# taki0112/vit-tensorflow

Hardware: AMD Instinct MI355X
Metric: images/sec (fwd+bwd) ViT-B/16 224px bf16 (higher is better)
Workload: dtype bf16; 1 GPU; vit_b16_224 fwd+bwd, batch 256/GPU, N(0,1) NHWC images resident in HBM, random-init weights, softmax-CE cotangent, dropout 0; global_batch=256, parallelism=dp1, compute=bf16

## Files before the change

### vit-tensorflow_amd/csrc/gemm_bf16.hip

```cpp
#include <array>
#include <map>
#include <mutex>

#include "gemm_bf16_common.h"

static int g_allow_320 = 1;
static int g_shared_gpu = 0;
int gemm_bf16_pick(int M, int N);

namespace {

template <int BM, int BN, int WM, int WN, int MODE, bool LDS_EPI, int SCHED>
__global__ __launch_bounds__(WM * WN * 64) void gemm_bf16_nt_kernel(Bf16GemmArgs g, EpiParams ep, int tiles_m, int tiles_n,
                                                                    int kt_per_split) {
  constexpr int NW = WM * WN;
  constexpr int WTM = BM / WM, WTN = BN / WN;
  constexpr int MT = WTM / 32, NT = WTN / 32;
  constexpr int A_BYTES = BM * BK * 2, B_BYTES = BN * BK * 2, STAGE = A_BYTES + B_BYTES;
  constexpr int A_INSTR = BM / 8 / NW, B_INSTR = BN / 8 / NW;
  static_assert(BM % (8 * NW) == 0 && BN % (8 * NW) == 0, "tile rows must split evenly over the waves");
  extern __shared__ __attribute__((aligned(16))) char smem[];

  const int nwg = gridDim.x, bid = blockIdx.x;
  const int xcd = bid & 7, q8 = nwg >> 3, r8 = nwg & 7;
// ... 8 lines not shown
  const int wave = __builtin_amdgcn_readfirstlane(tid >> 6);
  const int wm = wave / WN, wn = wave - wm * WN;

  if (g.stagger > 0 && bid < 256 && blockIdx.y == 0) {
    const int ph = (bid >> 3) & 3;
    for (int i = 0; i < ph * g.stagger; ++i) __builtin_amdgcn_s_sleep(32);
  }

  int offA[A_INSTR], offB[B_INSTR];
#pragma unroll
  for (int i = 0; i < A_INSTR; ++i) {
    const int row = (i * NW + wave) * 8 + (lane >> 3);
    const int c = (lane & 7) ^ ((row >> 1) & 7);
    offA[i] = row * (int)g.lda + c * 8;
  }
#pragma unroll
  for (int i = 0; i < B_INSTR; ++i) {
    const int row = (i * NW + wave) * 8 + (lane >> 3);
    const int c = (lane & 7) ^ ((row >> 1) & 7);
    offB[i] = row * (int)g.ldb + c * 8;
  }
  auto stage_ptr = [&](int buf, const bf16_t* Ap, const bf16_t* Bp, int kt) {
    char* base = smem + buf * STAGE;
#pragma unroll
    for (int i = 0; i < A_INSTR; ++i)
      __builtin_amdgcn_global_load_lds((gbl_void_t*)(Ap + (offA[i] + kt * BK)),
                                       (lds_void_t*)(base + (i * NW + wave) * 1024), 16, 0, 0);
#pragma unroll
    for (int i = 0; i < B_INSTR; ++i)
      __builtin_amdgcn_global_load_lds((gbl_void_t*)(Bp + (offB[i] + kt * BK)),
                                       (lds_void_t*)(base + A_BYTES + (i * NW + wave) * 1024), 16, 0, 0);
  };

  const int sw = ((lane & 31) >> 1) & 7;
  const int a_row_byte = (wm * WTM + (lane & 31)) * 128;
  const int b_row_byte = A_BYTES + (wn * WTN + (lane & 31)) * 128;
  const int khalf = lane >> 5;
  const bool has_bias = ep.bias != nullptr, has_scale = ep.scale != nullptr;
  const int64_t out_off = (int64_t)z * ep.partial_stride;

  int it = 0;
  int logical = logical0;
  if (logical >= total_tiles) return;
  const int gm = (tiles_n >= 8 ? 4 : 1) * (g.reverse_m ? -1 : 1);
  int tile_m, tile_n;
  decode_tile(logical, tiles_m, tiles_n, gm, tile_m, tile_n);
  const bf16_t* Ag = g.A + (int64_t)tile_m * BM * g.lda + (int64_t)kt0 * BK;
  const bf16_t* Bg = g.B + (int64_t)tile_n * BN * g.ldb + (int64_t)kt0 * BK;
  if (SCHED == 2 && nk > 0) stage_ptr(0, Ag, Bg, 0);

  for (;;) {
    auto stage = [&](int buf, int kt) { stage_ptr(buf, Ag, Bg, kt); };
    const int next_logical = logical + nwg;
    const bool has_next = SCHED == 2 && next_logical < total_tiles;
    int ntm = 0, ntn = 0;
    if (has_next) decode_tile(next_logical, tiles_m, tiles_n, gm, ntm, ntn);
    const bf16_t* Agn = g.A + (int64_t)ntm * BM * g.lda + (int64_t)kt0 * BK;
    const bf16_t* Bgn = g.B + (int64_t)ntn * BN * g.ldb + (int64_t)kt0 * BK;

    f32x16 acc[MT][NT];
#pragma unroll
    for (int i = 0; i < MT; ++i)
#pragma unroll
      for (int j = 0; j < NT; ++j)
#pragma unroll
        for (int r = 0; r < 16; ++r) acc[i][j][r] = 0.f;

    {
      if (SCHED != 2 && nk > 0) stage(0, 0);
      for (int kt = 0; kt < nk; ++kt) {
        asm volatile("s_waitcnt vmcnt(0)" ::: "memory");
        __syncthreads();
        if (kt + 1 < nk) stage((it + 1) & 1, kt + 1);
        else if (has_next) stage_ptr((it + 1) & 1, Agn, Bgn, 0);
        const char* base = smem + (it & 1) * STAGE;
#pragma unroll
        for (int ks = 0; ks < BK / 16; ++ks) {
          const int cb = ((ks * 2 + khalf) ^ sw) << 4;
          bf16x8 af[MT], bfr[NT];
#pragma unroll
          for (int i = 0; i < MT; ++i) af[i] = *(const bf16x8*)(base + a_row_byte + i * 32 * 128 + cb);
#pragma unroll
          for (int j = 0; j < NT; ++j) bfr[j] = *(const bf16x8*)(base + b_row_byte + j * 32 * 128 + cb);
#pragma unroll
          for (int i = 0; i < MT; ++i)
#pragma unroll
            for (int j = 0; j < NT; ++j)
              acc[i][j] = __builtin_amdgcn_mfma_f32_32x32x16_bf16(bfr[j], af[i], acc[i][j], 0, 0, 0);
        }
        ++it;
      }
    }

    const bool interior = epilogue_fast_ok(ep, MODE) && (tile_m + 1) * BM <= ep.M && (tile_n + 1) * BN <= ep.N;
    constexpr int RR = ((SCHED == 2 && 64 * (BN + 4) * 4 > STAGE) || (MT % 2 != 0)) ? 32 : 64;
    if constexpr (LDS_EPI) {
      constexpr int SROW = BN + 4;
      constexpr int LPRW = BN / 4, RPIW = 64 / LPRW;
      constexpr int RPW = RR / (NW * RPIW);
      static_assert(RPW >= 1 && RR * SROW * 4 <= (SCHED == 2 ? 1 : 2) * STAGE, "staging round must fit the free pipeline buffer(s)");
      float* st = (float*)(smem + (SCHED == 2 ? ((it + 1) & 1) * STAGE : 0));
      const int col_l = (lane % LPRW) * 4;
      const int gcol = tile_n * BN + col_l;
      float4 b4 = make_float4(0.f, 0.f, 0.f, 0.f), s4 = make_float4(1.f, 1.f, 1.f, 1.f);
      if (interior && has_bias) b4 = *(const float4*)(ep.bias + gcol);
      if (interior && has_scale) s4 = *(const float4*)(ep.scale + gcol);
      float4 cs = make_float4(0.f, 0.f, 0.f, 0.f);
      auto cs_add = [&](float4 r) { if (MODE == EPI_GELU_BWD) { cs.x += r.x; cs.y += r.y; cs.z += r.z; cs.w += r.w; } };
#pragma clang loop unroll(full)
      for (int R = 0; R < BM / RR; ++R) {
        const int wm_r = (R * RR) / WTM, i0 = ((R * RR) % WTM) / 32;
        __syncthreads();
        if (wm == wm_r) {
#pragma unroll
          for (int ii = 0; ii < RR / 32; ++ii)
#pragma unroll
            for (int j = 0; j < NT; ++j)
#pragma unroll
              for (int q = 0; q < 4; ++q)
                *(float4*)(st + (ii * 32 + (lane & 31)) * SROW + wn * WTN + j * 32 + 8 * q + 4 * khalf) =
                    make_float4(acc[i0 + ii][j][4 * q], acc[i0 + ii][j][4 * q + 1], acc[i0 + ii][j][4 * q + 2], acc[i0 + ii][j][4 * q + 3]);
        }
        __syncthreads();
        float4 v[RPW];
#pragma unroll
        for (int k = 0; k < RPW; ++k) v[k] = *(const float4*)(st + ((k * NW + wave) * RPIW + lane / LPRW) * SROW + col_l);
        const int grow0 = tile_m * BM + R * RR + lane / LPRW;
        if (interior) {
          float4 x[RPW];
#pragma unroll
          for (int k = 0; k < RPW; ++k) x[k] = epilogue_fast_load<MODE, bf16_t>(ep, grow0 + (k * NW + wave) * RPIW, gcol);
          if (MODE == EPI_BIAS_RESID && has_scale) {
#pragma unroll
            for (int k = 0; k < RPW; ++k) {
              if (has_bias) epilogue_fast4<MODE, bf16_t, true, true>(ep, grow0 + (k * NW + wave) * RPIW, gcol, v[k], b4, s4, x[k], out_off);
              else epilogue_fast4<MODE, bf16_t, false, true>(ep, grow0 + (k * NW + wave) * RPIW, gcol, v[k], b4, s4, x[k], out_off);
            }
          } else if (has_bias) {
#pragma unroll
            for (int k = 0; k < RPW; ++k) cs_add(epilogue_fast4<MODE, bf16_t, true, false>(ep, grow0 + (k * NW + wave) * RPIW, gcol, v[k], b4, s4, x[k], out_off));
          } else {
#pragma unroll
            for (int k = 0; k < RPW; ++k) cs_add(epilogue_fast4<MODE, bf16_t, false, false>(ep, grow0 + (k * NW + wave) * RPIW, gcol, v[k], b4, s4, x[k], out_off));
          }
        } else {
#pragma unroll
          for (int k = 0; k < RPW; ++k) cs_add(epilogue_apply4<MODE, bf16_t>(ep, grow0 + (k * NW + wave) * RPIW, gcol, v[k], out_off));
        }
      }
      if (MODE == EPI_GELU_BWD && ep.colsum != nullptr) {
        __syncthreads();
        *(float4*)(st + (wave * RPIW + lane / LPRW) * BN + col_l) = cs;
        __syncthreads();
        if (tid < BN) {
          float a = 0.f;
#pragma unroll
          for (int w = 0; w < NW * RPIW; ++w) a += st[w * BN + tid];
          const int c = tile_n * BN + tid;
          if (c < ep.N) ep.colsum[(int64_t)tile_m * ep.ldcs + c] = a;
        }
      }
      if (SCHED == 2) __syncthreads();
    } else {
      const int row0 = tile_m * BM + wm * WTM + (lane & 31);
      const int col00 = tile_n * BN + wn * WTN + 4 * khalf;
      if (interior) {
        auto run = [&](auto hb, auto hs) {
          constexpr bool HB = decltype(hb)::value, HS = decltype(hs)::value;
#pragma unroll
          for (int j = 0; j < NT; ++j)
#pragma unroll
            for (int qp = 0; qp < 2; ++qp) {
              float4 b4[2], s4[2], x[2][MT];
#pragma unroll
              for (int qq = 0; qq < 2; ++qq) {
                const int col = col00 + j * 32 + 8 * (2 * qp + qq);
                b4[qq] = HB ? *(const float4*)(ep.bias + col) : make_float4(0.f, 0.f, 0.f, 0.f);
                s4[qq] = HS ? *(const float4*)(ep.scale + col) : make_float4(1.f, 1.f, 1.f, 1.f);
#pragma unroll
                for (int i = 0; i < MT; ++i) x[qq][i] = epilogue_fast_load<MODE, bf16_t>(ep, row0 + i * 32, col);
              }
#pragma unroll
              for (int qq = 0; qq < 2; ++qq) {
                const int q = 2 * qp + qq;
                const int col = col00 + j * 32 + 8 * q;
#pragma unroll
                for (int i = 0; i < MT; ++i)
                  epilogue_fast4<MODE, bf16_t, HB, HS>(ep, row0 + i * 32, col,
                                                       make_float4(acc[i][j][4 * q], acc[i][j][4 * q + 1], acc[i][j][4 * q + 2], acc[i][j][4 * q + 3]),
                                                       b4[qq], s4[qq], x[qq][i], out_off);
              }
            }
        };
        if (has_bias && has_scale) run(std::true_type{}, std::true_type{});
        else if (has_bias) run(std::true_type{}, std::false_type{});
        else run(std::false_type{}, std::false_type{});
      } else {
#pragma unroll
        for (int i = 0; i < MT; ++i) {
#pragma unroll
          for (int j = 0; j < NT; ++j) {
#pragma unroll
            for (int q = 0; q < 4; ++q)
              epilogue_apply4<MODE, bf16_t>(ep, row0 + i * 32, col00 + j * 32 + 8 * q,
                                            make_float4(acc[i][j][4 * q], acc[i][j][4 * q + 1], acc[i][j][4 * q + 2], acc[i][j][4 * q + 3]),
                                            out_off);
          }
        }
      }
    }

    if (!has_next) break;
    logical = next_logical;
    tile_m = ntm; tile_n = ntn;
    Ag = Agn; Bg = Bgn;
  }
}

template <int BM, int BN, int WM, int WN, int MODE, bool LDS_EPI, int SCHED = 0>
void launch_variant(const Bf16GemmArgs& g, const EpiParams& ep, hipStream_t s) {
  constexpr int SMEM = 2 * (BM + BN) * BK * 2;
  static_assert(64 * (BN + 4) * 4 <= SMEM, "epilogue staging must fit in the pipeline buffers");
  auto kern = gemm_bf16_nt_kernel<BM, BN, WM, WN, MODE, LDS_EPI, SCHED>;
  vitx_set_max_smem((const void*)kern, SMEM);
  const int tiles_m = (int)ceil_div(g.M, BM), tiles_n = (int)ceil_div(g.N, BN);
  const int nk = g.K / BK;
  const int split = g.split_k > 1 ? g.split_k : 1;
  const int per = (int)ceil_div(nk, split);
  const int zs = (int)ceil_div(nk, per);
  const unsigned gx = (SCHED == 2 && zs == 1) ? (unsigned)std::min(tiles_m * tiles_n, 256) : (unsigned)(tiles_m * tiles_n);
  dim3 grid(gx, (unsigned)zs), block(WM * WN * 64);
  hipLaunchKernelGGL(kern, grid, block, SMEM, s, g, ep, tiles_m, tiles_n, per);
}

template <int MODE>
void launch_mode(const Bf16GemmArgs& g, const EpiParams& ep, hipStream_t s) {
  int k = g.kernel & 15;
  if (k == 0) k = gemm_bf16_pick(g.M, g.N);
  const bool bf16_out = (MODE == EPI_STORE || MODE == EPI_BIAS_GELU || MODE == EPI_GELU_BWD);
// ... 188 lines not shown
```

### vit-tensorflow_amd/csrc/gemm_bf16_common.h

```cpp
#pragma once
#include <algorithm>
#include <cstdio>
#include <cstdlib>
#include <type_traits>
#include <utility>

#include "kernels.h"

namespace {

typedef __attribute__((address_space(3))) void lds_void_t;
typedef const __attribute__((address_space(1))) void gbl_void_t;

constexpr int BK = 64;

template <typename F, int... I>
__device__ __forceinline__ void static_for_impl(F&& f, std::integer_sequence<int, I...>) { (f(std::integral_constant<int, I>{}), ...); }
template <int N, typename F>
__device__ __forceinline__ void static_for(F&& f) { static_for_impl(f, std::make_integer_sequence<int, N>{}); }
template <int V> using ic = std::integral_constant<int, V>;

__device__ __forceinline__ void decode_tile_fwd(int L, int tiles_m, int tiles_n, int gm, int& tm, int& tn);
__device__ __forceinline__ void decode_tile(int L, int tiles_m, int tiles_n, int gm, int& tm, int& tn) {
  if (gm < 0) { decode_tile_fwd(L, tiles_m, tiles_n, -gm, tm, tn); tm = tiles_m - 1 - tm; return; }
  decode_tile_fwd(L, tiles_m, tiles_n, gm, tm, tn);
}
__device__ __forceinline__ void decode_tile_fwd(int L, int tiles_m, int tiles_n, int gm, int& tm, int& tn) {
  if (gm == 1) { tm = L / tiles_n; tn = L - tm * tiles_n; return; }
  const int group = gm * tiles_n;
  const int gid = L / group, first = gid * gm;
  const int gsz = min(tiles_m - first, gm);
  const int w = L - gid * group;
  tn = w / gsz;
  tm = first + (w - tn * gsz);
}

}

void launch_gemm_bf16_pipe(int variant, int mode, const Bf16GemmArgs& g, const EpiParams& ep, hipStream_t s);
int gemm_bf16_shared_gpu();
void launch_gemm_bf16_persistent_lockstep(int bm, int mode, const Bf16GemmArgs& g, const EpiParams& ep, hipStream_t s);
```

### vit-tensorflow_amd/csrc/gemm_bf16_pipe.hip

```cpp
#include "gemm_bf16_common.h"

#include <cmath>
#include <cstring>
#include <map>
#include <mutex>
#include <vector>

namespace {

__device__ __forceinline__ int wp_lane() {
  int l;
  asm volatile("v_mbcnt_lo_u32_b32 %0, -1, 0\n\tv_mbcnt_hi_u32_b32 %0, -1, %0" : "=v"(l));
  return l;
}

template <int POL>
__device__ __forceinline__ void wp_store16(bf16_t* base, uint32_t elem_off, bf16x8 v) {
  if constexpr (POL == 1) __builtin_nontemporal_store(v, (bf16x8*)(base + elem_off));
  else *(bf16x8*)(base + elem_off) = v;
}

constexpr int GT_LO = (127 - 12) << 7, GT_NE = ((127 + 3) << 7) - GT_LO, GT_BYTES = 2 * GT_NE * 4;
const uint32_t* gelu_table_dev() {
  static std::mutex mu;
  static std::map<int, const uint32_t*> per_dev;
  int dev = 0;
  (void)hipGetDevice(&dev);
  std::lock_guard<std::mutex> lk(mu);
  auto it = per_dev.find(dev);
  if (it != per_dev.end()) return it->second;
  std::vector<uint32_t> h((size_t)2 * GT_NE);
  auto f32_to_bf16 = [](float f) { uint32_t u; memcpy(&u, &f, 4); u += 0x7fffu + ((u >> 16) & 1u); return (uint16_t)(u >> 16); };
  auto f32_to_f16 = [](float f) { _Float16 hh = (_Float16)f; uint16_t u; memcpy(&u, &hh, 2); return u; };
  for (int sgn = 0; sgn < 2; ++sgn)
    for (int t = 0; t < GT_NE; ++t) {
      const uint32_t bits = ((uint32_t)sgn << 31) | ((uint32_t)(t + GT_LO) << 16);
      float xf; memcpy(&xf, &bits, 4);
      const double x = xf, phi = 0.5 * (1.0 + erf(x * 0.70710678118654752440)), gd = phi + x * 0.39894228040143267794 * exp(-0.5 * x * x);
      h[(size_t)sgn * GT_NE + t] = ((uint32_t)f32_to_f16((float)phi) << 16) | f32_to_bf16((float)gd);
    }
  uint32_t* d = nullptr;
  if (hipMalloc((void**)&d, GT_BYTES) != hipSuccess || hipMemcpy(d, h.data(), GT_BYTES, hipMemcpyHostToDevice) != hipSuccess) d = nullptr;
  per_dev[dev] = d;
  return d;
}

// ... 46 lines not shown
  for (int i = 0; i < B_INSTR; ++i) {
    const int row = (wave * B_INSTR + i) * 8 + (lane >> 3);
    offB[i] = (uint32_t)(row * (int)g.ldb + (((lane & 7) ^ ((row >> 1) & 7)) << 3)) * 2u - (uint32_t)((i & 3) * 1024);
  }

  const int gm = ((tiles_n >= 8 && g.stagger != 8) ? 4 : 1) * (g.reverse_m ? -1 : 1);
  auto tile_of = [&](int idx, int& tm, int& tn) {
    if (xw) {
      decode_tile_fwd(idx, w_nr, tiles_n, 8, tm, tn);
      tm += w_r0;
      if (g.reverse_m) tm = tiles_m - 1 - tm;
    } else {
      decode_tile(idx, tiles_m, tiles_n, gm, tm, tn);
    }
  };
  int i_logical = w_first, i_k = 0, issued = 0;
  bool i_more = nk > 0;
  const i32x4 rsA = vitx_make_rsrc(g.A), rsB = vitx_make_rsrc(g.B);
  const uint32_t lds_wa = vitx_lds_addr(smem) + (uint32_t)wave * (A_INSTR * 1024u);
  const uint32_t lds_wb = vitx_lds_addr(smem) + A_BYTES + (uint32_t)wave * (B_INSTR * 1024u);
  uint32_t a_soff = 0, b_soff = 0;
  auto i_set_tile = [&]() {
    int tm, tn;
    tile_of(i_logical, tm, tn);
    a_soff = (uint32_t)(((int64_t)tm * BM * g.lda + (int64_t)kt0 * BK) * 2);
    b_soff = (uint32_t)(((int64_t)tn * BN * g.ldb + (int64_t)kt0 * BK) * 2);
    {
      a_soff = (uint32_t)__builtin_amdgcn_readfirstlane((int)a_soff);
      b_soff = (uint32_t)__builtin_amdgcn_readfirstlane((int)b_soff);
    }
  };
  i_set_tile();
  constexpr int P = A_INSTR + B_INSTR;
  constexpr int N3 = (P + 2) / 3;
  constexpr int N0 = (P + 1) / 3;
  constexpr int N1 = P - N3 - N0;
  bool pending = false;
  const int xp = g.stagger;
  auto issue_piece = [&](uint32_t base, auto p_c) {
    constexpr int p = decltype(p_c)::value;
    const uint32_t sa = a_soff + i_k * (BK * 2), sb = b_soff + i_k * (BK * 2), lb = base;
    if constexpr (p < A_INSTR) {
      if constexpr ((p & 3) == 0) vitx_dma16(rsA, lds_wa + lb + p * 1024, offA[p], sa);
      else vitx_dma16_cont<(p & 3) * 1024>(rsA, offA[p], sa);
    } else {
      constexpr int q = p - A_INSTR;
      if constexpr ((q & 3) == 0) vitx_dma16(rsB, lds_wb + lb + q * 1024, offB[q], sb);
      else vitx_dma16_cont<(q & 3) * 1024>(rsB, offB[q], sb);
    }
  };
  auto i_advance = [&]() {
    ++issued;
    if (++i_k == nk) {
      i_k = 0;
      i_logical += w_stride;
      i_more = persistent && i_logical < w_limit;
      if (i_more) i_set_tile();
    }
  };
  auto issue = [&]() {
    if (!i_more) return;
    const uint32_t base = (issued & 1) * STAGE;
    static_for<P>([&](auto p_c) { issue_piece(base, p_c); });
    i_advance();
  };

  const int sw = ((lane & 31) >> 1) & 7;
  const int a_row_byte = (wm * WTM + (lane & 31)) * 128;
  const int b_row_byte = A_BYTES + (wn * WTN + (lane & 31)) * 128;
  const int khalf = lane >> 5;
  bf16x8 fa[2][MT], fb[2][NT];
  auto load_frags = [&](bf16x8(&af)[MT], bf16x8(&bfr)[NT], const char* base, int ks) {
    const int cb = ((ks * 2 + khalf) ^ sw) << 4;
#pragma unroll
    for (int i = 0; i < MT; ++i) af[i] = *(const bf16x8*)(base + a_row_byte + i * 32 * 128 + cb);
#pragma unroll
    for (int j = 0; j < NT; ++j) bfr[j] = *(const bf16x8*)(base + b_row_byte + j * 32 * 128 + cb);
  };
  constexpr int Q = MT * NT;
  f32x16 acc[MT][NT];
  auto mfma_range = [&](auto cur_c, auto first_c, auto last_c) {
    constexpr int CUR = decltype(cur_c)::value, FIRST = decltype(first_c)::value, LAST = decltype(last_c)::value;
    static_for<(LAST > FIRST ? LAST - FIRST : 0)>([&](auto d) {
      constexpr int idx = FIRST + decltype(d)::value, i = idx / NT, j = idx % NT;
      acc[i][j] = __builtin_amdgcn_mfma_f32_32x32x16_bf16(fb[CUR][j], fa[CUR][i], acc[i][j], 0, 0, 0);
    });
  };
  auto handover = [&]() {
    if (xp & 1) __builtin_amdgcn_s_waitcnt(0xC07F);
    else __builtin_amdgcn_s_waitcnt(0x0070);
    __builtin_amdgcn_s_barrier();
    asm volatile("" ::: "memory");
  };
  const bool has_bias = ep.bias != nullptr, has_scale = ep.scale != nullptr;
  const int64_t out_off = (int64_t)z * ep.partial_stride;

  issue();
  issue();
  constexpr bool GTAB = MODE == EPI_BIAS_GELU && BM == 256;
  if constexpr (GTAB) {
    if (gelu_tab != nullptr) {
      uint32_t* t = (uint32_t*)(smem + 2 * STAGE);
      for (int i = tid; i < 2 * GT_NE; i += NW * 64) t[i] = gelu_tab[i];
    }
  }
  handover();
  load_frags(fa[0], fb[0], smem, 0);
  int it = 0;
  int tile_idx = 0;
#ifndef VITX_GEMM_STAMPS_BUILD
#define VITX_GEMM_STAMPS_BUILD 0
#endif
  constexpr bool kStamps = VITX_GEMM_STAMPS_BUILD != 0;
  auto stamp = [&](int k) {
    if constexpr (kStamps)
      if (g.stamps && tid == 0 && bid < 512 && tile_idx < 15) {
        g.stamps[((int64_t)bid * 16 + tile_idx) * 4 + k] = __builtin_readcyclecounter();
        if (tile_idx == 0 && k == 0)
          g.stamps[((int64_t)bid * 16 + 15) * 4] = ((unsigned long long)__builtin_amdgcn_s_getreg((31 << 11) | 20) << 32) | (unsigned)__builtin_amdgcn_s_getreg((31 << 11) | 4);
      }
  };
  for (int logical = w_first;; logical += w_stride, ++tile_idx) {
    int tile_m, tile_n;
    tile_of(logical, tile_m, tile_n);
    const bool has_next = persistent && logical + w_stride < w_limit;
    stamp(0);
#pragma unroll
    for (int i = 0; i < MT; ++i)
#pragma unroll
      for (int j = 0; j < NT; ++j)
#pragma unroll
        for (int r = 0; r < 16; ++r) acc[i][j][r] = 0.f;

    for (int kt = 0; kt < nk; ++kt) {
      const char* base = smem + (it & 1) * STAGE;
      static_for<BK / 16>([&](auto ks_c) {
        constexpr int ks = decltype(ks_c)::value, CUR = ks & 1;
        constexpr int NP = ks == 3 ? N3 : (ks == 0 ? N0 : (ks == 1 ? N1 : 0));
        constexpr int FP = ks == 3 ? 0 : (ks == 0 ? N3 : N3 + N0);
        if constexpr (ks + 1 < BK / 16) {
          mfma_range(ic<CUR>{}, ic<0>{}, ic<2>{});
          __builtin_amdgcn_sched_barrier(0);
          if (!(xp & 4)) load_frags(fa[CUR ^ 1], fb[CUR ^ 1], base, ks + 1);
        } else {
          handover();
          mfma_range(ic<CUR>{}, ic<0>{}, ic<2>{});
          __builtin_amdgcn_sched_barrier(0);
          if (kt + 1 < nk && !(xp & 4)) load_frags(fa[0], fb[0], smem + ((it + 1) & 1) * STAGE, 0);
          pending = i_more && kt + 1 < nk && !(xp & 2);
        }
        __builtin_amdgcn_sched_barrier(0);
        if constexpr (NP > 0) {
          const uint32_t ibase = (issued & 1) * STAGE;
          static_for<NP>([&](auto d_c) {
            constexpr int d = decltype(d_c)::value;
            mfma_range(ic<CUR>{}, ic<(2 + d < Q ? 2 + d : Q)>{}, ic<(3 + d < Q ? 3 + d : Q)>{});
            if (pending) issue_piece(ibase, ic<FP + d>{});
            __builtin_amdgcn_sched_barrier(0);
          });
          mfma_range(ic<CUR>{}, ic<(2 + NP < Q ? 2 + NP : Q)>{}, ic<Q>{});
          if constexpr (FP + NP == P) {
            if (pending) i_advance();
            pending = false;
          }
        } else {
          mfma_range(ic<CUR>{}, ic<2>{}, ic<Q>{});
        }
        __builtin_amdgcn_sched_barrier(0);
      });
      ++it;
    }

    stamp(1);
    bool wp_done = false;
    {
      const bool interior = epilogue_fast_ok(ep, MODE) && (tile_m + 1) * BM <= ep.M && (tile_n + 1) * BN <= ep.N;
      static_assert((BM == 256 || BM == 320 || BM == 192) && A_INSTR >= 4 && B_INSTR == 4 && WTN == 64 && MT * 32 == WTM && NT == 2, "wave-private epilogue: 256 / 320 x 256 tiles, 2 x 4 waves");
      if constexpr (MODE == EPI_STORE || MODE == EPI_BIAS_GELU || MODE == EPI_BIAS_RESID || MODE == EPI_GELU_BWD) {
        const bool wp_ok = interior && (MODE == EPI_BIAS_RESID || ep.wide_ok) && !(MODE == EPI_STORE && has_bias);
        if (wp_ok) {
          wp_done = true;
          char* const sa = smem + ((it + 1) & 1) * STAGE + wave * (A_INSTR * 1024);
          char* const sb = smem + ((it + 1) & 1) * STAGE + A_BYTES + wave * (B_INSTR * 1024);
          const int le = wp_lane();
          const int m = le & 31, swm = (m >> 1) & 7, kh = le >> 5;
          const int row_w = tile_m * BM + wm * WTM, col_w = tile_n * BN + wn * WTN;
          auto to_bf16x4 = [](float a, float b, float c, float d) { bf16x4 o; o[0] = (bf16_t)a; o[1] = (bf16_t)b; o[2] = (bf16_t)c; o[3] = (bf16_t)d; return o; };
          auto stage_f32 = [&](auto i_c) {
            constexpr int i0 = decltype(i_c)::value;
#pragma unroll
            for (int q = 0; q < 4; ++q) {
              const int ch = 2 * q + kh;
              *(float4*)(sa + m * 128 + ((ch ^ swm) << 4)) = make_float4(acc[i0][0][4 * q], acc[i0][0][4 * q + 1], acc[i0][0][4 * q + 2], acc[i0][0][4 * q + 3]);
              *(float4*)(sb + (m ^ 1) * 128 + ((ch ^ swm ^ 1) << 4)) = make_float4(acc[i0][1][4 * q], acc[i0][1][4 * q + 1], acc[i0][1][4 * q + 2], acc[i0][1][4 * q + 3]);
            }
          };
          if constexpr (MODE == EPI_STORE) {
            bf16_t* const outp = (bf16_t*)ep.out + out_off + (int64_t)row_w * ep.ldo + col_w;
            const uint32_t ldo = (uint32_t)ep.ldo, ooff = (uint32_t)(le >> 3) * ldo + (uint32_t)(le & 7) * 8u;
            auto run = [&](auto nt_c) {
              constexpr int POL = decltype(nt_c)::value;
              static_for<MT>([&](auto i_c) {
                constexpr int i0 = decltype(i_c)::value;
                char* const ar = (i0 & 1) ? sb : sa;
#pragma unroll
                for (int j = 0; j < NT; ++j)
#pragma unroll
                  for (int q = 0; q < 4; ++q)
                    *(bf16x4*)(ar + m * 128 + (((j * 4 + q) ^ swm) << 4) + kh * 8) =
                        to_bf16x4(acc[i0][j][4 * q], acc[i0][j][4 * q + 1], acc[i0][j][4 * q + 2], acc[i0][j][4 * q + 3]);
                bf16x8 v[4];
#pragma unroll
                for (int k = 0; k < 4; ++k) {
                  const int r = k * 8 + (le >> 3);
                  v[k] = *(const bf16x8*)(ar + r * 128 + (((le & 7) ^ ((r >> 1) & 7)) << 4));
                }
#pragma unroll
                for (int k = 0; k < 4; ++k) wp_store16<POL>(outp, ooff + (uint32_t)(i0 * 32 + k * 8) * ldo, v[k]);
              });
            };
            if (ep.nt_out) run(ic<1>{});
            else run(ic<0>{});
          } else if constexpr (MODE == EPI_BIAS_GELU) {
            const float* const bias_w = has_bias ? ep.bias + col_w + 4 * kh : nullptr;
            bf16_t* const o1 = (bf16_t*)ep.out + (int64_t)row_w * ep.ldo + col_w;
            bf16_t* const o2 = (bf16_t*)ep.out2 + (int64_t)row_w * ep.ldo2 + col_w;
            const uint32_t ldo = (uint32_t)ep.ldo, ldo2 = (uint32_t)ep.ldo2;
            const uint32_t o1off = (uint32_t)(le >> 3) * ldo + (uint32_t)(le & 7) * 8u, o2off = (uint32_t)(le >> 3) * ldo2 + (uint32_t)(le & 7) * 8u;
            const bool use_tab = GTAB && gelu_tab != nullptr;
            const char* const gt = smem + 2 * STAGE;
            auto run = [&](auto nt_c, auto tab_c) {
              constexpr int POL = decltype(nt_c)::value;
              constexpr bool TAB = decltype(tab_c)::value;
              static_for<MT>([&](auto i_c) {
                constexpr int i0 = decltype(i_c)::value;
#pragma unroll
                for (int j = 0; j < NT; ++j) {
                  float4 bzj[4];
#pragma unroll
                  for (int q = 0; q < 4; ++q) bzj[q] = bias_w ? *(const float4*)(bias_w + j * 32 + 8 * q) : make_float4(0.f, 0.f, 0.f, 0.f);
#pragma unroll
                  for (int q = 0; q < 4; ++q) {
                    const bf16x4 h = to_bf16x4(acc[i0][j][4 * q] + bzj[q].x, acc[i0][j][4 * q + 1] + bzj[q].y, acc[i0][j][4 * q + 2] + bzj[q].z,
                                               acc[i0][j][4 * q + 3] + bzj[q].w);
                    const int off = m * 128 + (((j * 4 + q) ^ swm) << 4) + kh * 8;
                    if constexpr (TAB) {
                      const uint32_t p0 = __builtin_bit_cast(uint2, h).x, p1 = __builtin_bit_cast(uint2, h).y;
                      auto look = [&](uint32_t bits15, uint32_t sign) {
                        const int t = min(max((int)bits15 - GT_LO, 0), GT_NE - 1);
                        return *(const uint32_t*)(gt + ((uint32_t)t + sign * GT_NE) * 4u);
                      };
                      const uint32_t e0 = look(p0 & 0x7fffu, (p0 >> 15) & 1u), e1 = look((p0 >> 16) & 0x7fffu, p0 >> 31);
                      const uint32_t e2 = look(p1 & 0x7fffu, (p1 >> 15) & 1u), e3 = look((p1 >> 16) & 0x7fffu, p1 >> 31);
                      auto phi = [](uint32_t e) { return (float)__builtin_bit_cast(_Float16, (uint16_t)(e >> 16)); };
                      const float x0 = __builtin_bit_cast(float, p0 << 16), x1 = __builtin_bit_cast(float, p0 & 0xffff0000u);
                      const float x2 = __builtin_bit_cast(float, p1 << 16), x3 = __builtin_bit_cast(float, p1 & 0xffff0000u);
                      uint2 gdw;
                      gdw.x = __builtin_amdgcn_perm(e1, e0, 0x05040100u);
                      gdw.y = __builtin_amdgcn_perm(e3, e2, 0x05040100u);
                      *(uint2*)(sa + off) = gdw;
                      *(bf16x4*)(sb + off) = to_bf16x4(x0 * phi(e0), x1 * phi(e1), x2 * phi(e2), x3 * phi(e3));
                    } else {
                      float4 g, gd;
                      gelu_both4(make_float4((float)h[0], (float)h[1], (float)h[2], (float)h[3]), g, gd);
                      *(bf16x4*)(sa + off) = to_bf16x4(gd.x, gd.y, gd.z, gd.w);
                      *(bf16x4*)(sb + off) = to_bf16x4(g.x, g.y, g.z, g.w);
                    }
                  }
                }
                bf16x8 vd[4], vg[4];
#pragma unroll
                for (int k = 0; k < 4; ++k) {
                  const int r = k * 8 + (le >> 3);
                  const int off = r * 128 + (((le & 7) ^ ((r >> 1) & 7)) << 4);
                  vd[k] = *(const bf16x8*)(sa + off);
                  vg[k] = *(const bf16x8*)(sb + off);
                }
#pragma unroll
                for (int k = 0; k < 4; ++k) {
                  wp_store16<POL>(o1, o1off + (uint32_t)(i0 * 32 + k * 8) * ldo, vd[k]);
                  wp_store16<0>(o2, o2off + (uint32_t)(i0 * 32 + k * 8) * ldo2, vg[k]);
                }
              });
            };
            if constexpr (GTAB) {
              if (use_tab) { if (ep.nt_out) run(ic<1>{}, std::true_type{}); else run(ic<0>{}, std::true_type{}); }
              else if (ep.nt_out) run(ic<1>{}, std::false_type{});
              else run(ic<0>{}, std::false_type{});
            } else {
              if (ep.nt_out) run(ic<1>{}, std::false_type{});
              else run(ic<0>{}, std::false_type{});
            }
          } else if constexpr (MODE == EPI_BIAS_RESID) {
            const int c16 = le & 15, ar1 = c16 >> 3;
            const uint32_t lr = (uint32_t)(le >> 4), lc = (uint32_t)c16 * 4u;
            const float4 bb = has_bias ? *(const float4*)(ep.bias + col_w + lc) : make_float4(0.f, 0.f, 0.f, 0.f);
            const float4 ss = has_scale ? *(const float4*)(ep.scale + col_w + lc) : make_float4(1.f, 1.f, 1.f, 1.f);
            const char* const rb = ar1 ? sb : sa;
            const float* const rp = ep.resid + (int64_t)row_w * ep.ldr + col_w;
// ... 49 lines not shown
                const char* rowp = rb + (r ^ ar1) * 128;
                const int swr = ((r >> 1) & 7) ^ ar1;
                va[k] = *(const float4*)(rowp + ((ch0 ^ swr) << 4));
                vb[k] = *(const float4*)(rowp + (((ch0 + 1) ^ swr) << 4));
              }
#pragma unroll
              for (int k = 0; k < 4; ++k) {
                const float4 a = va[k], b = vb[k];
                const bf16x8 o = pack_bf16x8(make_float4(a.x * (float)x[k][0], a.y * (float)x[k][1], a.z * (float)x[k][2], a.w * (float)x[k][3]),
                                             make_float4(b.x * (float)x[k][4], b.y * (float)x[k][5], b.z * (float)x[k][6], b.w * (float)x[k][7]));
                wp_store16<0>(op, ooff + (uint32_t)(i0 * 32 + k * 8) * ldo, o);
                cs.x += (float)o[0]; cs.y += (float)o[1]; cs.z += (float)o[2]; cs.w += (float)o[3];
                cs2.x += (float)o[4]; cs2.y += (float)o[5]; cs2.z += (float)o[6]; cs2.w += (float)o[7];
              }
            });
            if (ep.colsum != nullptr) {
              auto red = [&](float v) { v += __shfl_xor(v, 8); v += __shfl_xor(v, 16); v += __shfl_xor(v, 32); return v; };
              cs.x = red(cs.x); cs.y = red(cs.y); cs.z = red(cs.z); cs.w = red(cs.w);
              cs2.x = red(cs2.x); cs2.y = red(cs2.y); cs2.z = red(cs2.z); cs2.w = red(cs2.w);
              if (le < 8) {
                float* crow = ep.colsum + (int64_t)(tile_m * 2 + wm) * ep.ldcs + col_w + lc;
                *(float4*)crow = cs;
                *(float4*)(crow + 4) = cs2;
              }
            }
          }
        }
      }
      {
        if (!wp_done) {
          const int le = wp_lane();
          char* const sa = smem + ((it + 1) & 1) * STAGE + wave * (A_INSTR * 1024);
          char* const sb = smem + ((it + 1) & 1) * STAGE + A_BYTES + wave * (B_INSTR * 1024);
          const int m = le & 31, swm = (m >> 1) & 7, kh = le >> 5;
          const int row_w = tile_m * BM + wm * WTM, col_w = tile_n * BN + wn * WTN;
          const int c16 = le & 15, ar1 = c16 >> 3, lr = le >> 4, gcolr = col_w + c16 * 4;
          const char* const rb = ar1 ? sb : sa;
          float4 cs = make_float4(0.f, 0.f, 0.f, 0.f);
          static_for<MT>([&](auto i_c) {
            constexpr int i0 = decltype(i_c)::value;
#pragma unroll
            for (int q = 0; q < 4; ++q) {
              const int ch = 2 * q + kh;
              *(float4*)(sa + m * 128 + ((ch ^ swm) << 4)) = make_float4(acc[i0][0][4 * q], acc[i0][0][4 * q + 1], acc[i0][0][4 * q + 2], acc[i0][0][4 * q + 3]);
              *(float4*)(sb + (m ^ 1) * 128 + ((ch ^ swm ^ 1) << 4)) = make_float4(acc[i0][1][4 * q], acc[i0][1][4 * q + 1], acc[i0][1][4 * q + 2], acc[i0][1][4 * q + 3]);
            }
#pragma unroll 2
            for (int k = 0; k < 8; ++k) {
              const int r = k * 4 + lr;
              const float4 v = *(const float4*)(rb + (r ^ ar1) * 128 + ((((c16 & 7) ^ ((r >> 1) & 7)) ^ ar1) << 4));
              const float4 res = epilogue_apply4<MODE, bf16_t>(ep, row_w + i0 * 32 + r, gcolr, v, out_off);
              if (MODE == EPI_GELU_BWD) { cs.x += res.x; cs.y += res.y; cs.z += res.z; cs.w += res.w; }
            }
          });
          if (MODE == EPI_GELU_BWD && ep.colsum != nullptr) {
            auto red = [&](float v) { v += __shfl_xor(v, 16); v += __shfl_xor(v, 32); return v; };
            cs.x = red(cs.x); cs.y = red(cs.y); cs.z = red(cs.z); cs.w = red(cs.w);
            if (le < 16 && gcolr < ep.N) {
              float* crow = ep.colsum + (int64_t)(tile_m * 2 + wm) * ep.ldcs + gcolr;
              if (gcolr + 3 < ep.N) *(float4*)crow = cs;
              else { crow[0] = cs.x; if (gcolr + 1 < ep.N) crow[1] = cs.y; if (gcolr + 2 < ep.N) crow[2] = cs.z; }
            }
          }
        }
      }

    }
    stamp(2);
    if (!has_next) break;
    __builtin_amdgcn_s_waitcnt(0xC07F);
    asm volatile("" ::: "memory");
    issue();
    load_frags(fa[0], fb[0], smem + (it & 1) * STAGE, 0);
    stamp(3);
  }
}

template <int BM, int BN, int WM, int WN, int MODE>
void launch_pipe(const Bf16GemmArgs& g, const EpiParams& ep, hipStream_t s, bool one_tile_per_wg = false) {
  constexpr int SMEM = 2 * (BM + BN) * BK * 2 + ((MODE == EPI_BIAS_GELU && BM == 256) ? GT_BYTES : 0);
  if (((int64_t)ceil_div(g.M, BM) * BM * g.lda + g.K) * 2 >= (1LL << 31) || ((int64_t)ceil_div(g.N, BN) * BN * g.ldb + g.K) * 2 >= (1LL << 31)) {
    launch_gemm_bf16_persistent_lockstep(BM, MODE, g, ep, s);
    return;
  }
  auto kern = gemm_bf16_nt_pipe_kernel<BM, BN, WM, WN, MODE>;
  vitx_set_max_smem((const void*)kern, SMEM);
  const int tiles_m = (int)ceil_div(g.M, BM), tiles_n = (int)ceil_div(g.N, BN);
  const int nk = g.K / BK;
  const int split = g.split_k > 1 ? g.split_k : 1;
  const int per = (int)ceil_div(nk, split);
  const int zs = (int)ceil_div(nk, per);
  static const int phase_env = [] { const char* v = vitx_env("VITX_GEMM_PHASE"); return v ? atoi(v) : 0; }();
  Bf16GemmArgs gp = g;
  if (gp.phase == 0) gp.phase = phase_env;
  static const int walk_env = [] { const char* v = vitx_env("VITX_GEMM_WALK"); return v ? atoi(v) : -1; }();
  static const int grid_cap = [] { const char* v = vitx_env("VITX_GEMM_GRID"); return v ? atoi(v) : 256 * (WM * WN == 4 ? 2 : 1); }();
  const unsigned gx = (zs == 1 && !gemm_bf16_shared_gpu() && !g.shared_gpu && !one_tile_per_wg) ? (unsigned)std::min(tiles_m * tiles_n, grid_cap) : (unsigned)(tiles_m * tiles_n);
  dim3 grid(gx, (unsigned)zs), block(WM * WN * 64);
  const bool walk2_ok = BM == 256 && zs == 1 && gx == (unsigned)grid_cap && (gx & 7) == 0 && gx < (unsigned)(tiles_m * tiles_n) && tiles_n >= 8 && tiles_m >= 64 && g.stagger != 8;
  gp.walk = (walk2_ok && walk_env != 0) ? 2 : 0;
  const uint32_t* gtab = (MODE == EPI_BIAS_GELU && BM == 256 && gelu_table_on()) ? gelu_table_dev() : nullptr;
  hipLaunchKernelGGL(kern, grid, block, SMEM, s, gp, ep, tiles_m, tiles_n, per, gtab);
}

template <int MODE>
void pipe_mode(int variant, const Bf16GemmArgs& g, const EpiParams& ep, hipStream_t s) {
// ... 25 lines not shown
```

Before: 7620 images/sec.

## Switch bf16 NT GEMM kernels from 32x32x16 to 16x16x32 MFMA

Replaces the 32x32x16 bf16 MFMA instruction with 16x16x32 MFMA in both the basic and pipelined NT GEMM kernels. Each 32x32 accumulator is kept as four 16x16 sub-blocks, and LDS fragment loads are recomputed for 16-row groups with a quarter-K lane split. The pipelined kernel's interleaving of global-to-LDS pieces and fragment reloads is rescheduled around two half passes over the tile. Epilogue and staging offsets now go through an acc_pos abstraction for the new accumulator layout. The aim is higher MFMA throughput or better latency hiding, at the cost of more LDS reads per K step, more issue slots, and schedule complexity.

```diff
diff --git a/vit-tensorflow_amd/csrc/gemm_bf16.hip b/vit-tensorflow_amd/csrc/gemm_bf16.hip
--- a/vit-tensorflow_amd/csrc/gemm_bf16.hip
+++ b/vit-tensorflow_amd/csrc/gemm_bf16.hip
@@ -64,10 +64,10 @@
                                        (lds_void_t*)(base + A_BYTES + (i * NW + wave) * 1024), 16, 0, 0);
   };
 
-  const int sw = ((lane & 31) >> 1) & 7;
-  const int a_row_byte = (wm * WTM + (lane & 31)) * 128;
-  const int b_row_byte = A_BYTES + (wn * WTN + (lane & 31)) * 128;
-  const int khalf = lane >> 5;
+  const int sw = ((lane & 15) >> 1) & 7;
+  const int a_row_byte = (wm * WTM + (lane & 15)) * 128;
+  const int b_row_byte = A_BYTES + (wn * WTN + (lane & 15)) * 128;
+  const int kq = lane >> 4;
   const bool has_bias = ep.bias != nullptr, has_scale = ep.scale != nullptr;
   const int64_t out_off = (int64_t)z * ep.partial_stride;
 
@@ -106,20 +106,19 @@
         if (kt + 1 < nk) stage((it + 1) & 1, kt + 1);
         else if (has_next) stage_ptr((it + 1) & 1, Agn, Bgn, 0);
         const char* base = smem + (it & 1) * STAGE;
-#pragma unroll
-        for (int ks = 0; ks < BK / 16; ++ks) {
-          const int cb = ((ks * 2 + khalf) ^ sw) << 4;
-          bf16x8 af[MT], bfr[NT];
-#pragma unroll
-          for (int i = 0; i < MT; ++i) af[i] = *(const bf16x8*)(base + a_row_byte + i * 32 * 128 + cb);
-#pragma unroll
-          for (int j = 0; j < NT; ++j) bfr[j] = *(const bf16x8*)(base + b_row_byte + j * 32 * 128 + cb);
-#pragma unroll
-          for (int i = 0; i < MT; ++i)
-#pragma unroll
-            for (int j = 0; j < NT; ++j)
-              acc[i][j] = __builtin_amdgcn_mfma_f32_32x32x16_bf16(bfr[j], af[i], acc[i][j], 0, 0, 0);
-        }
+        static_for<BK / 32>([&](auto ks_c) {
+          constexpr int ks = decltype(ks_c)::value;
+          const int cb = ((ks * 4 + kq) ^ sw) << 4;
+          bf16x8 af[2 * MT], bfr[2 * NT];
+#pragma unroll
+          for (int i = 0; i < 2 * MT; ++i) af[i] = *(const bf16x8*)(base + a_row_byte + i * 16 * 128 + cb);
+#pragma unroll
+          for (int j = 0; j < 2 * NT; ++j) bfr[j] = *(const bf16x8*)(base + b_row_byte + j * 16 * 128 + cb);
+          static_for<4 * MT * NT>([&](auto d) {
+            constexpr int b16 = decltype(d)::value / (2 * NT), j16 = decltype(d)::value % (2 * NT);
+            mfma_item<(b16 & 1) * 2 + (j16 & 1)>(acc[b16 >> 1][j16 >> 1], bfr[j16], af[b16]);
+          });
+        });
         ++it;
       }
     }
@@ -149,9 +148,10 @@
 #pragma unroll
             for (int j = 0; j < NT; ++j)
 #pragma unroll
-              for (int q = 0; q < 4; ++q)
-                *(float4*)(st + (ii * 32 + (lane & 31)) * SROW + wn * WTN + j * 32 + 8 * q + 4 * khalf) =
-                    make_float4(acc[i0 + ii][j][4 * q], acc[i0 + ii][j][4 * q + 1], acc[i0 + ii][j][4 * q + 2], acc[i0 + ii][j][4 * q + 3]);
+              for (int q = 0; q < 4; ++q) {
+                const vitx_acc::Pos p = acc_pos(lane, q);
+                *(float4*)(st + (ii * 32 + p.row) * SROW + wn * WTN + j * 32 + p.col) = acc_item(acc[i0 + ii][j], q);
+              }
         }
         __syncthreads();
         float4 v[RPW];
@@ -194,8 +194,7 @@
       }
       if (SCHED == 2) __syncthreads();
     } else {
-      const int row0 = tile_m * BM + wm * WTM + (lane & 31);
-      const int col00 = tile_n * BN + wn * WTN + 4 * khalf;
+      const int row_w = tile_m * BM + wm * WTM, col_w = tile_n * BN + wn * WTN;
       if (interior) {
         auto run = [&](auto hb, auto hs) {
           constexpr bool HB = decltype(hb)::value, HS = decltype(hs)::value;
@@ -206,21 +205,21 @@
               float4 b4[2], s4[2], x[2][MT];
 #pragma unroll
               for (int qq = 0; qq < 2; ++qq) {
-                const int col = col00 + j * 32 + 8 * (2 * qp + qq);
+                const vitx_acc::Pos p = acc_pos(lane, 2 * qp + qq);
+                const int col = col_w + j * 32 + p.col;
                 b4[qq] = HB ? *(const float4*)(ep.bias + col) : make_float4(0.f, 0.f, 0.f, 0.f);
                 s4[qq] = HS ? *(const float4*)(ep.scale + col) : make_float4(1.f, 1.f, 1.f, 1.f);
 #pragma unroll
-                for (int i = 0; i < MT; ++i) x[qq][i] = epilogue_fast_load<MODE, bf16_t>(ep, row0 + i * 32, col);
+                for (int i = 0; i < MT; ++i) x[qq][i] = epilogue_fast_load<MODE, bf16_t>(ep, row_w + i * 32 + p.row, col);
               }
 #pragma unroll
               for (int qq = 0; qq < 2; ++qq) {
                 const int q = 2 * qp + qq;
-                const int col = col00 + j * 32 + 8 * q;
+                const vitx_acc::Pos p = acc_pos(lane, q);
+                const int col = col_w + j * 32 + p.col;
 #pragma unroll
                 for (int i = 0; i < MT; ++i)
-                  epilogue_fast4<MODE, bf16_t, HB, HS>(ep, row0 + i * 32, col,
-                                                       make_float4(acc[i][j][4 * q], acc[i][j][4 * q + 1], acc[i][j][4 * q + 2], acc[i][j][4 * q + 3]),
-                                                       b4[qq], s4[qq], x[qq][i], out_off);
+                  epilogue_fast4<MODE, bf16_t, HB, HS>(ep, row_w + i * 32 + p.row, col, acc_item(acc[i][j], q), b4[qq], s4[qq], x[qq][i], out_off);
               }
             }
         };
@@ -233,10 +232,10 @@
 #pragma unroll
           for (int j = 0; j < NT; ++j) {
 #pragma unroll
-            for (int q = 0; q < 4; ++q)
-              epilogue_apply4<MODE, bf16_t>(ep, row0 + i * 32, col00 + j * 32 + 8 * q,
-                                            make_float4(acc[i][j][4 * q], acc[i][j][4 * q + 1], acc[i][j][4 * q + 2], acc[i][j][4 * q + 3]),
-                                            out_off);
+            for (int q = 0; q < 4; ++q) {
+              const vitx_acc::Pos p = acc_pos(lane, q);
+              epilogue_apply4<MODE, bf16_t>(ep, row_w + i * 32 + p.row, col_w + j * 32 + p.col, acc_item(acc[i][j], q), out_off);
+            }
           }
         }
       }
diff --git a/vit-tensorflow_amd/csrc/gemm_bf16_acc.h b/vit-tensorflow_amd/csrc/gemm_bf16_acc.h
--- /dev/null
+++ b/vit-tensorflow_amd/csrc/gemm_bf16_acc.h
@@ -0,0 +1,20 @@
+#pragma once
+
+namespace vitx_acc {
+
+struct Pos { int row, col; };
+
+template <int SHAPE>
+constexpr Pos acc_pos(int lane, int q) {
+  static_assert(SHAPE == 16 || SHAPE == 32, "MFMA shapes of the bf16 NT family");
+  if constexpr (SHAPE == 32) return Pos{lane & 31, 8 * q + 4 * (lane >> 5)};
+  else return Pos{16 * (q >> 1) + (lane & 15), 16 * (q & 1) + 4 * (lane >> 4)};
+}
+
+template <int SHAPE>
+constexpr Pos acc_tile_pos(int lane, int i, int j, int q) {
+  const Pos p = acc_pos<SHAPE>(lane, q);
+  return Pos{32 * i + p.row, 32 * j + p.col};
+}
+
+}
diff --git a/vit-tensorflow_amd/csrc/gemm_bf16_common.h b/vit-tensorflow_amd/csrc/gemm_bf16_common.h
--- a/vit-tensorflow_amd/csrc/gemm_bf16_common.h
+++ b/vit-tensorflow_amd/csrc/gemm_bf16_common.h
@@ -5,6 +5,7 @@
 #include <type_traits>
 #include <utility>
 
+#include "gemm_bf16_acc.h"
 #include "kernels.h"
 
 namespace {
@@ -13,6 +14,17 @@
 typedef const __attribute__((address_space(1))) void gbl_void_t;
 
 constexpr int BK = 64;
+
+constexpr int NT_MFMA = 16;
+__device__ __forceinline__ vitx_acc::Pos acc_pos(int lane, int q) { return vitx_acc::acc_pos<NT_MFMA>(lane, q); }
+__device__ __forceinline__ float4 acc_item(const f32x16& a, int q) { return make_float4(a[4 * q], a[4 * q + 1], a[4 * q + 2], a[4 * q + 3]); }
+template <int Q>
+__device__ __forceinline__ void mfma_item(f32x16& a, bf16x8 bfrag, bf16x8 afrag) {
+  f32x4 c;
+  c[0] = a[4 * Q]; c[1] = a[4 * Q + 1]; c[2] = a[4 * Q + 2]; c[3] = a[4 * Q + 3];
+  c = __builtin_amdgcn_mfma_f32_16x16x32_bf16(bfrag, afrag, c, 0, 0, 0);
+  a[4 * Q] = c[0]; a[4 * Q + 1] = c[1]; a[4 * Q + 2] = c[2]; a[4 * Q + 3] = c[3];
+}
 
 template <typename F, int... I>
 __device__ __forceinline__ void static_for_impl(F&& f, std::integer_sequence<int, I...>) { (f(std::integral_constant<int, I>{}), ...); }
diff --git a/vit-tensorflow_amd/csrc/gemm_bf16_pipe.hip b/vit-tensorflow_amd/csrc/gemm_bf16_pipe.hip
--- a/vit-tensorflow_amd/csrc/gemm_bf16_pipe.hip
+++ b/vit-tensorflow_amd/csrc/gemm_bf16_pipe.hip
@@ -12,6 +12,22 @@
   int l;
   asm volatile("v_mbcnt_lo_u32_b32 %0, -1, 0\n\tv_mbcnt_hi_u32_b32 %0, -1, %0" : "=v"(l));
   return l;
+}
+
+__device__ __forceinline__ int stage_f32_off(int lane, int q, int area) {
+  const vitx_acc::Pos p = acc_pos(lane, q);
+  return (p.row ^ area) * 128 + ((((p.col >> 2) ^ ((p.row >> 1) & 7)) ^ area) << 4);
+}
+__device__ __forceinline__ int stage_bf16_off(int lane, int j, int q) {
+  const vitx_acc::Pos p = acc_pos(lane, q);
+  const int c = 32 * j + p.col;
+  return p.row * 128 + (((c >> 3) ^ ((p.row >> 1) & 7)) << 4) + ((c >> 2) & 1) * 8;
+}
+
+constexpr int piece_behind(int idx, int h, int np) {
+  for (int d = 0; d < np; ++d)
+    if ((d + 1) * h / (np + 1) - 1 == idx) return d;
+  return -1;
 }
 
 template <int POL>
@@ -124,9 +140,6 @@
   };
   i_set_tile();
   constexpr int P = A_INSTR + B_INSTR;
-  constexpr int N3 = (P + 2) / 3;
-  constexpr int N0 = (P + 1) / 3;
-  constexpr int N1 = P - N3 - N0;
   bool pending = false;
   const int xp = g.stagger;
   auto issue_piece = [&](uint32_t base, auto p_c) {
@@ -157,30 +170,45 @@
     i_advance();
   };
 
-  const int sw = ((lane & 31) >> 1) & 7;
-  const int a_row_byte = (wm * WTM + (lane & 31)) * 128;
-  const int b_row_byte = A_BYTES + (wn * WTN + (lane & 31)) * 128;
-  const int khalf = lane >> 5;
-  bf16x8 fa[2][MT], fb[2][NT];
-  auto load_frags = [&](bf16x8(&af)[MT], bf16x8(&bfr)[NT], const char* base, int ks) {
-    const int cb = ((ks * 2 + khalf) ^ sw) << 4;
-#pragma unroll
-    for (int i = 0; i < MT; ++i) af[i] = *(const bf16x8*)(base + a_row_byte + i * 32 * 128 + cb);
-#pragma unroll
-    for (int j = 0; j < NT; ++j) bfr[j] = *(const bf16x8*)(base + b_row_byte + j * 32 * 128 + cb);
-  };
-  constexpr int Q = MT * NT;
+  const int sw16 = ((lane & 15) >> 1) & 7, kq = lane >> 4;
+  const int a_row16 = (wm * WTM + (lane & 15)) * 128, b_row16 = A_BYTES + (wn * WTN + (lane & 15)) * 128;
+  bf16x8 xa[2][MT], xb[2 * NT];
+  auto load_a16 = [&](bf16x8(&af)[MT], const char* base, int ks, int half) {
+    const int cb = ((ks * 4 + kq) ^ sw16) << 4;
+#pragma unroll
+    for (int i = 0; i < MT; ++i) af[i] = *(const bf16x8*)(base + a_row16 + (half * MT + i) * 16 * 128 + cb);
+  };
+  auto load_b16 = [&](bf16x8& bfr, const char* base, int ks, int j16) {
+    bfr = *(const bf16x8*)(base + b_row16 + j16 * 16 * 128 + (((ks * 4 + kq) ^ sw16) << 4));
+  };
   f32x16 acc[MT][NT];
-  auto mfma_range = [&](auto cur_c, auto first_c, auto last_c) {
-    constexpr int CUR = decltype(cur_c)::value, FIRST = decltype(first_c)::value, LAST = decltype(last_c)::value;
-    static_for<(LAST > FIRST ? LAST - FIRST : 0)>([&](auto d) {
-      constexpr int idx = FIRST + decltype(d)::value, i = idx / NT, j = idx % NT;
-      acc[i][j] = __builtin_amdgcn_mfma_f32_32x32x16_bf16(fb[CUR][j], fa[CUR][i], acc[i][j], 0, 0, 0);
+  constexpr int H16 = MT * 2 * NT;
+  auto mfma16_half = [&](auto half_c, auto np_c, auto fp_c, const char* nbase, int nks, bool reload) {
+    constexpr int HALF = decltype(half_c)::value, NPC = decltype(np_c)::value, FPC = decltype(fp_c)::value;
+    const uint32_t ibase = (issued & 1) * STAGE;
+    static_for<H16>([&](auto x_c) {
+      constexpr int idx = decltype(x_c)::value, j16 = idx / MT, bi = idx % MT, b16 = HALF * MT + bi;
+      mfma_item<(b16 & 1) * 2 + (j16 & 1)>(acc[b16 >> 1][j16 >> 1], xb[j16], xa[HALF][bi]);
+      if constexpr (HALF == 1 && bi == MT - 1) {
+        __builtin_amdgcn_sched_barrier(0);
+        if (reload) load_b16(xb[j16], nbase, nks, j16);
+        __builtin_amdgcn_sched_barrier(0);
+      }
+      constexpr int d = piece_behind(idx, H16, NPC);
+      if constexpr (d >= 0) {
+        if (pending) issue_piece(ibase, ic<FPC + d>{});
+        __builtin_amdgcn_sched_barrier(0);
+      }
     });
-  };
+    if constexpr (NPC > 0 && FPC + NPC == P) {
+      if (pending) i_advance();
+      pending = false;
+    }
+  };
+  constexpr int PA = (P + 2) / 3, PB = (P - PA + 1) / 2, PC = P - PA - PB;
   auto handover = [&]() {
-    if (xp & 1) __builtin_amdgcn_s_waitcnt(0xC07F);
-    else __builtin_amdgcn_s_waitcnt(0x0070);
+    __builtin_amdgcn_s_waitcnt(0xC07F);
+    if (!(xp & 1)) __builtin_amdgcn_s_waitcnt(0x0F70);
     __builtin_amdgcn_s_barrier();
     asm volatile("" ::: "memory");
   };
@@ -197,7 +225,13 @@
     }
   }
   handover();
-  load_frags(fa[0], fb[0], smem, 0);
+  auto first_frags = [&](const char* base) {
+    load_a16(xa[0], base, 0, 0);
+#pragma unroll
+    for (int j = 0; j < 2 * NT; ++j) load_b16(xb[j], base, 0, j);
+    load_a16(xa[1], base, 0, 1);
+  };
+  first_frags(smem);
   int it = 0;
   int tile_idx = 0;
 #ifndef VITX_GEMM_STAMPS_BUILD
@@ -226,40 +260,26 @@
 
     for (int kt = 0; kt < nk; ++kt) {
       const char* base = smem + (it & 1) * STAGE;
-      static_for<BK / 16>([&](auto ks_c) {
-        constexpr int ks = decltype(ks_c)::value, CUR = ks & 1;
-        constexpr int NP = ks == 3 ? N3 : (ks == 0 ? N0 : (ks == 1 ? N1 : 0));
-        constexpr int FP = ks == 3 ? 0 : (ks == 0 ? N3 : N3 + N0);
-        if constexpr (ks + 1 < BK / 16) {
-          mfma_range(ic<CUR>{}, ic<0>{}, ic<2>{});
-          __builtin_amdgcn_sched_barrier(0);
-          if (!(xp & 4)) load_frags(fa[CUR ^ 1], fb[CUR ^ 1], base, ks + 1);
-        } else {
-          handover();
-          mfma_range(ic<CUR>{}, ic<0>{}, ic<2>{});
-          __builtin_amdgcn_sched_barrier(0);
-          if (kt + 1 < nk && !(xp & 4)) load_frags(fa[0], fb[0], smem + ((it + 1) & 1) * STAGE, 0);
-          pending = i_more && kt + 1 < nk && !(xp & 2);
-        }
-        __builtin_amdgcn_sched_barrier(0);
-        if constexpr (NP > 0) {
-          const uint32_t ibase = (issued & 1) * STAGE;
-          static_for<NP>([&](auto d_c) {
-            constexpr int d = decltype(d_c)::value;
-            mfma_range(ic<CUR>{}, ic<(2 + d < Q ? 2 + d : Q)>{}, ic<(3 + d < Q ? 3 + d : Q)>{});
-            if (pending) issue_piece(ibase, ic<FP + d>{});
-            __builtin_amdgcn_sched_barrier(0);
-          });
-          mfma_range(ic<CUR>{}, ic<(2 + NP < Q ? 2 + NP : Q)>{}, ic<Q>{});
-          if constexpr (FP + NP == P) {
-            if (pending) i_advance();
-            pending = false;
-          }
-        } else {
-          mfma_range(ic<CUR>{}, ic<2>{}, ic<Q>{});
-        }
-        __builtin_amdgcn_sched_barrier(0);
-      });
+      mfma16_half(ic<0>{}, ic<PB>{}, ic<PA>{}, base, 1, false);
+      __builtin_amdgcn_sched_barrier(0);
+      if (!(xp & 4)) load_a16(xa[0], base, 1, 0);
+      __builtin_amdgcn_sched_barrier(0);
+      mfma16_half(ic<1>{}, ic<PC>{}, ic<PA + PB>{}, base, 1, !(xp & 4));
+      __builtin_amdgcn_sched_barrier(0);
+      if (!(xp & 4)) load_a16(xa[1], base, 1, 1);
+      __builtin_amdgcn_sched_barrier(0);
+      mfma16_half(ic<0>{}, ic<0>{}, ic<0>{}, base, 1, false);
+      __builtin_amdgcn_sched_barrier(0);
+      handover();
+      const char* nbase = smem + ((it + 1) & 1) * STAGE;
+      const bool nfrags = kt + 1 < nk && !(xp & 4);
+      if (nfrags) load_a16(xa[0], nbase, 0, 0);
+      pending = i_more && kt + 1 < nk && !(xp & 2);
+      __builtin_amdgcn_sched_barrier(0);
+      mfma16_half(ic<1>{}, ic<PA>{}, ic<0>{}, nbase, 0, nfrags);
+      __builtin_amdgcn_sched_barrier(0);
+      if (nfrags) load_a16(xa[1], nbase, 0, 1);
+      __builtin_amdgcn_sched_barrier(0);
       ++it;
     }
 
@@ -275,16 +295,14 @@
           char* const sa = smem + ((it + 1) & 1) * STAGE + wave * (A_INSTR * 1024);
           char* const sb = smem + ((it + 1) & 1) * STAGE + A_BYTES + wave * (B_INSTR * 1024);
           const int le = wp_lane();
-          const int m = le & 31, swm = (m >> 1) & 7, kh = le >> 5;
           const int row_w = tile_m * BM + wm * WTM, col_w = tile_n * BN + wn * WTN;
-          auto to_bf16x4 = [](float a, float b, float c, float d) { bf16x4 o; o[0] = (bf16_t)a; o[1] = (bf16_t)b; o[2] = (bf16_t)c; o[3] = (bf16_t)d; return o; };
+          auto to_bf16x4 = [](float4 v) { bf16x4 o; o[0] = (bf16_t)v.x; o[1] = (bf16_t)v.y; o[2] = (bf16_t)v.z; o[3] = (bf16_t)v.w; return o; };
           auto stage_f32 = [&](auto i_c) {
             constexpr int i0 = decltype(i_c)::value;
 #pragma unroll
             for (int q = 0; q < 4; ++q) {
-              const int ch = 2 * q + kh;
-              *(float4*)(sa + m * 128 + ((ch ^ swm) << 4)) = make_float4(acc[i0][0][4 * q], acc[i0][0][4 * q + 1], acc[i0][0][4 * q + 2], acc[i0][0][4 * q + 3]);
-              *(float4*)(sb + (m ^ 1) * 128 + ((ch ^ swm ^ 1) << 4)) = make_float4(acc[i0][1][4 * q], acc[i0][1][4 * q + 1], acc[i0][1][4 * q + 2], acc[i0][1][4 * q + 3]);
+              *(float4*)(sa + stage_f32_off(le, q, 0)) = acc_item(acc[i0][0], q);
+              *(float4*)(sb + stage_f32_off(le, q, 1)) = acc_item(acc[i0][1], q);
             }
           };
           if constexpr (MODE == EPI_STORE) {
@@ -299,8 +317,7 @@
                 for (int j = 0; j < NT; ++j)
 #pragma unroll
                   for (int q = 0; q < 4; ++q)
-                    *(bf16x4*)(ar + m * 128 + (((j * 4 + q) ^ swm) << 4) + kh * 8) =
-                        to_bf16x4(acc[i0][j][4 * q], acc[i0][j][4 * q + 1], acc[i0][j][4 * q + 2], acc[i0][j][4 * q + 3]);
+                    *(bf16x4*)(ar + stage_bf16_off(le, j, q)) = to_bf16x4(acc_item(acc[i0][j], q));
                 bf16x8 v[4];
 #pragma unroll
                 for (int k = 0; k < 4; ++k) {
@@ -314,7 +331,7 @@
             if (ep.nt_out) run(ic<1>{});
             else run(ic<0>{});
           } else if constexpr (MODE == EPI_BIAS_GELU) {
-            const float* const bias_w = has_bias ? ep.bias + col_w + 4 * kh : nullptr;
+            const float* const bias_w = has_bias ? ep.bias + col_w : nullptr;
             bf16_t* const o1 = (bf16_t*)ep.out + (int64_t)row_w * ep.ldo + col_w;
             bf16_t* const o2 = (bf16_t*)ep.out2 + (int64_t)row_w * ep.ldo2 + col_w;
             const uint32_t ldo = (uint32_t)ep.ldo, ldo2 = (uint32_t)ep.ldo2;
@@ -328,14 +345,15 @@
                 constexpr int i0 = decltype(i_c)::value;
 #pragma unroll
                 for (int j = 0; j < NT; ++j) {
-                  float4 bzj[4];
-#pragma unroll
-                  for (int q = 0; q < 4; ++q) bzj[q] = bias_w ? *(const float4*)(bias_w + j * 32 + 8 * q) : make_float4(0.f, 0.f, 0.f, 0.f);
+                  constexpr int NBZ = NT_MFMA == 16 ? 2 : 4;
+                  float4 bzj[NBZ];
+#pragma unroll
+                  for (int q = 0; q < NBZ; ++q) bzj[q] = bias_w ? *(const float4*)(bias_w + j * 32 + acc_pos(le, q).col) : make_float4(0.f, 0.f, 0.f, 0.f);
 #pragma unroll
                   for (int q = 0; q < 4; ++q) {
-                    const bf16x4 h = to_bf16x4(acc[i0][j][4 * q] + bzj[q].x, acc[i0][j][4 * q + 1] + bzj[q].y, acc[i0][j][4 * q + 2] + bzj[q].z,
-                                               acc[i0][j][4 * q + 3] + bzj[q].w);
-                    const int off = m * 128 + (((j * 4 + q) ^ swm) << 4) + kh * 8;
+                    const float4 a = acc_item(acc[i0][j], q), bz = bzj[q % NBZ];
+                    const bf16x4 h = to_bf16x4(make_float4(a.x + bz.x, a.y + bz.y, a.z + bz.z, a.w + bz.w));
+                    const int off = stage_bf16_off(le, j, q);
                     if constexpr (TAB) {
                       const uint32_t p0 = __builtin_bit_cast(uint2, h).x, p1 = __builtin_bit_cast(uint2, h).y;
                       auto look = [&](uint32_t bits15, uint32_t sign) {
@@ -351,12 +369,12 @@
                       gdw.x = __builtin_amdgcn_perm(e1, e0, 0x05040100u);
                       gdw.y = __builtin_amdgcn_perm(e3, e2, 0x05040100u);
                       *(uint2*)(sa + off) = gdw;
-                      *(bf16x4*)(sb + off) = to_bf16x4(x0 * phi(e0), x1 * phi(e1), x2 * phi(e2), x3 * phi(e3));
+                      *(bf16x4*)(sb + off) = to_bf16x4(make_float4(x0 * phi(e0), x1 * phi(e1), x2 * phi(e2), x3 * phi(e3)));
                     } else {
                       float4 g, gd;
                       gelu_both4(make_float4((float)h[0], (float)h[1], (float)h[2], (float)h[3]), g, gd);
-                      *(bf16x4*)(sa + off) = to_bf16x4(gd.x, gd.y, gd.z, gd.w);
-                      *(bf16x4*)(sb + off) = to_bf16x4(g.x, g.y, g.z, g.w);
+                      *(bf16x4*)(sa + off) = to_bf16x4(gd);
+                      *(bf16x4*)(sb + off) = to_bf16x4(g);
                     }
                   }
                 }
@@ -472,7 +490,6 @@
           const int le = wp_lane();
           char* const sa = smem + ((it + 1) & 1) * STAGE + wave * (A_INSTR * 1024);
           char* const sb = smem + ((it + 1) & 1) * STAGE + A_BYTES + wave * (B_INSTR * 1024);
-          const int m = le & 31, swm = (m >> 1) & 7, kh = le >> 5;
           const int row_w = tile_m * BM + wm * WTM, col_w = tile_n * BN + wn * WTN;
           const int c16 = le & 15, ar1 = c16 >> 3, lr = le >> 4, gcolr = col_w + c16 * 4;
           const char* const rb = ar1 ? sb : sa;
@@ -481,9 +498,8 @@
             constexpr int i0 = decltype(i_c)::value;
 #pragma unroll
             for (int q = 0; q < 4; ++q) {
-              const int ch = 2 * q + kh;
-              *(float4*)(sa + m * 128 + ((ch ^ swm) << 4)) = make_float4(acc[i0][0][4 * q], acc[i0][0][4 * q + 1], acc[i0][0][4 * q + 2], acc[i0][0][4 * q + 3]);
-              *(float4*)(sb + (m ^ 1) * 128 + ((ch ^ swm ^ 1) << 4)) = make_float4(acc[i0][1][4 * q], acc[i0][1][4 * q + 1], acc[i0][1][4 * q + 2], acc[i0][1][4 * q + 3]);
+              *(float4*)(sa + stage_f32_off(le, q, 0)) = acc_item(acc[i0][0], q);
+              *(float4*)(sb + stage_f32_off(le, q, 1)) = acc_item(acc[i0][1], q);
             }
 #pragma unroll 2
             for (int k = 0; k < 8; ++k) {
@@ -511,7 +527,7 @@
     __builtin_amdgcn_s_waitcnt(0xC07F);
     asm volatile("" ::: "memory");
     issue();
-    load_frags(fa[0], fb[0], smem + (it & 1) * STAGE, 0);
+    first_frags(smem + (it & 1) * STAGE);
     stamp(3);
   }
 }
```

Result: no change. 7621 images/sec, median of 2 (+0.0%).
